# octaviogarcia/RaytracingOneWeekend

Hardware: AMD Instinct MI355X
Metric: Msamples/s (W×H×spp/s) + achieved HBM GB/s, 1080p@512spp traced scene (higher is better)
Workload: dtype f32; 1 GPU; C1 S-traced 1920x1080, 10496 spp timed (128 spp/step), depth 50; width=1920, height=1080, max_depth=50, parallelism=tile1, gather=RCCL send/recv (om_gather_frame), rccl_library=/usr/local/lib/python3.10/dist-packages/torch/lib/librccl.so, kernel=auto, pipeline=auto, tail_bounce=default, streams=2

## Files before the change

### raytracingoneweekend_amd/csrc/om_deal.h

```cpp
#pragma once
#include <cstdint>

#if defined(__HIPCC__) || defined(__CUDACC__)
#define OM_DEAL_HD __host__ __device__
#else
#define OM_DEAL_HD
#endif

struct Deal {
    uint64_t paths;
    uint64_t blocks;
    uint32_t nseg;
    uint32_t d;

    OM_DEAL_HD uint64_t groups() const { return (blocks + d - 1u) / d; }
    OM_DEAL_HD uint32_t blocks_of(uint32_t g) const {
        const uint64_t ng = groups();
        if (g >= ng) return 0u;
        const uint64_t mine = (ng - 1u - g) / nseg + 1u;
        uint64_t b = mine * d;
        if ((ng - 1u) % nseg == g) b -= ng * d - blocks;
        return (uint32_t)b;
    }
    OM_DEAL_HD uint64_t block(uint32_t g, uint32_t c) const {
        return ((uint64_t)(c / d) * nseg + g) * d + c % d;
    }
    OM_DEAL_HD uint32_t paths_of(uint32_t g) const {
        uint64_t n = (uint64_t)blocks_of(g) * 64u;
        if (blocks && ((blocks - 1u) / d) % nseg == g) n -= blocks * 64u - paths;
        return (uint32_t)n;
    }
    OM_DEAL_HD uint32_t capacity() const {
        return (uint32_t)((groups() + nseg - 1u) / nseg * d * 64u);
    }
};

inline uint32_t deal_segments(uint64_t max_paths, uint32_t cus, uint32_t lanes_per_cu, uint32_t blk, uint32_t spb) {
    const uint64_t want = (max_paths + blk - 1u) / blk, cap = (uint64_t)cus * (lanes_per_cu / blk);
    const uint32_t nseg = (uint32_t)(want < cap ? want : cap);
    return (nseg + spb - 1u) / spb * spb;
}

OM_DEAL_HD inline Deal make_deal(uint64_t paths, uint32_t nseg, uint32_t d) {
    return Deal{paths, (paths + 63u) / 64u, nseg, d};
}
```

### raytracingoneweekend_amd/csrc/om_tuning.h

```cpp
#pragma once

#ifndef OM_WF_BLOCK
#define OM_WF_BLOCK 512
#endif
#ifndef OM_WF_WAVES
#define OM_WF_WAVES 8
#endif
#ifndef OM_WF_TAIL_SPB
#define OM_WF_TAIL_SPB 2
#endif
#ifndef OM_WF_TAIL_WGS_PER_CU
#define OM_WF_TAIL_WGS_PER_CU 1
#endif
#ifndef OM_WF_MAX_PATHS_LOG2
#define OM_WF_MAX_PATHS_LOG2 27
#endif
#ifndef OM_WF_BATCH_SPP
#define OM_WF_BATCH_SPP 16
#endif
#ifndef OM_WF_MIN_PATHS_LOG2
#define OM_WF_MIN_PATHS_LOG2 25
#endif
#ifndef OM_WF_HYB_BYTES
#define OM_WF_HYB_BYTES 16384
#endif
#ifndef OM_WF_HYBW_BYTES
#define OM_WF_HYBW_BYTES 0
#endif
#ifndef OM_WF_HYB4_BYTES
#define OM_WF_HYB4_BYTES 0
#endif
#ifndef OM_WF_REFILL
#define OM_WF_REFILL 16
#endif
#ifndef OM_WF_TAIL_SHADE
#define OM_WF_TAIL_SHADE 1
#endif
#ifndef OM_WF_TAIL_UNROLL
#define OM_WF_TAIL_UNROLL 24
#endif
#ifndef OM_WF_TAIL_MARCH_WAVES
#define OM_WF_TAIL_MARCH_WAVES 8
#endif
#ifndef OM_WF_TAIL_REFILL
#define OM_WF_TAIL_REFILL OM_WF_REFILL
#endif
#ifndef OM_WF_TAIL_MARCHED
#define OM_WF_TAIL_MARCHED 1
#endif
#ifndef OM_MARCH_UNROLL
#define OM_MARCH_UNROLL 8
#endif
#ifndef OM_WF_ADAPTIVE_BATCHES
#define OM_WF_ADAPTIVE_BATCHES 3
#endif
#ifndef OM_WF_ADAPTIVE_PATHS_LOG2
#define OM_WF_ADAPTIVE_PATHS_LOG2 22
#endif
#ifndef OM_WF_ADAPTIVE_CAP_LOG2
#define OM_WF_ADAPTIVE_CAP_LOG2 26
#endif
#ifndef OM_WF_ADAPTIVE_TAIL
#define OM_WF_ADAPTIVE_TAIL 8
#endif
#ifndef OM_WF_LANES_PER_CU
#define OM_WF_LANES_PER_CU 2048
#endif
#ifndef OM_WF_LANES_PER_CU_WIDE
#define OM_WF_LANES_PER_CU_WIDE 8192
#endif
#ifndef OM_WF_DEAL_BLOCKS
#define OM_WF_DEAL_BLOCKS 8
#endif
#ifndef OM_WF_FUSE_B1
#define OM_WF_FUSE_B1 1
#endif
#ifndef OM_ACC_GROUP
#define OM_ACC_GROUP 8
#endif
#ifndef OM_B2_NODE_STRIDE
#define OM_B2_NODE_STRIDE 80
#endif
#ifndef OM_BARY_TREE_MIN
#define OM_BARY_TREE_MIN 16
#endif
#ifndef OM_SLAB_REACH
#define OM_SLAB_REACH 8192.0f
#endif
#ifndef OM_SPHERE_REACH
#define OM_SPHERE_REACH 16.0
#endif
```

### raytracingoneweekend_amd/csrc/om_wavefront.hip

```cpp
#include "om_wavefront.h"

#include <algorithm>
#include <type_traits>

#include "om_device.h"
#include "om_trace.h"
#include "om_tuning.h"
#include "om_deal.h"

using namespace omd;

namespace omw {

void QueueSet::release() {
    for (int a = 0; a < 2; ++a) {
        for (int b = 0; b < 3; ++b) { if (q[a][b]) (void)hipFree(q[a][b]); q[a][b] = nullptr; }
        if (qr[a]) (void)hipFree(qr[a]); qr[a] = nullptr;
    }
    if (res) (void)hipFree(res);
    if (res_id) (void)hipFree(res_id);
    if (counts) (void)hipFree(counts);
    if (hit) (void)hipFree(hit);
    res = nullptr; res_id = nullptr; counts = nullptr; hit = nullptr;
}

void Buffers::release() {
    for (auto& s : set) s.release();
    if (n0) (void)hipFree(n0);
    n0 = nullptr; n0_cap = 0;
    for (auto& st : side) { if (st) (void)hipStreamDestroy(st); st = nullptr; }

    for (auto e : ev) (void)hipEventDestroy(e);
    ev.clear();
    cap = 0; counts_n = 0; nsets = 0;
}

namespace {

constexpr uint32_t kNoSample = 0xFFFFFFFFu;
enum { TR_BRUTE = 1, TR_CULLED = 2, TR_BVH = 3, TR_SBVH_LDS = 4, TR_SBVH_GLOBAL = 5, TR_BVH2_LDS = 6, TR_BVH2_GLOBAL = 7,
       TR_BVH4_LDS = 8, TR_BVH4_GLOBAL = 9,
       TR_BVH2_WIDE = 10,
       TR_BARY = 16 };
constexpr int tr_base(int tr) { return tr & (TR_BARY - 1); }
constexpr bool tr_bary(int tr) { return (tr & TR_BARY) != 0; }
#define OM_WAVES_ATTR __attribute__((amdgpu_waves_per_eu(OM_WF_WAVES, OM_WF_WAVES)))
constexpr int kBlk = OM_WF_BLOCK;
constexpr int kStackDepth = 24;
constexpr uint32_t kB2Stride = OM_B2_NODE_STRIDE;
static_assert(kB2Stride % 16u == 0u && kB2Stride >= sizeof(OmBvh2Node), "16-B aligned node slots");
static_assert(kB2LdsBudget / sizeof(OmBvh2Node) * (kB2Stride / 16u) < OM_LEAF, "scaled BVH2 child codes stay below OM_LEAF");
template <int TR>
__host__ __device__ inline uint32_t stack_bytes(const OmSceneDev& S) {
    if (tr_base(TR) == TR_BVH2_WIDE) return kBlk * S.b2w_stack * 4u;
    return kBlk * ((tr_base(TR) == TR_BVH4_LDS || tr_base(TR) == TR_BVH4_GLOBAL) ? S.b4_stack : S.b2_stack) * 2u;
}
__host__ __device__ inline uint32_t b2_stage_bytes(const OmSceneDev& S) {
    return (S.n_b2nodes * kB2Stride + S.n_b2leaves * 4u + 15u) & ~15u;
}
constexpr uint32_t kTailSpb = OM_WF_TAIL_SPB;
constexpr uint32_t kTailWgsPerCu = OM_WF_TAIL_WGS_PER_CU;
constexpr uint32_t kWaves = kBlk / 64;
static_assert(kBlk % 64 == 0 && kTailWgsPerCu >= 1u, "whole waves; a tail grid");
constexpr bool kFuseB1 = OM_WF_FUSE_B1 != 0;
constexpr uint32_t kTailDefault = 16;
constexpr uint32_t kTailMarched = OM_WF_TAIL_MARCHED;
constexpr uint32_t kTailL2 = 10;
constexpr uint32_t kTailBigBatch = 24;
__host__ __device__ inline uint32_t hyb_nodes(const OmSceneDev& S) {
    constexpr uint32_t kCap = OM_WF_HYB_BYTES / (uint32_t)sizeof(OmBvh2NodeH);
    return S.b2_lds_bytes ? 0u : (S.n_b2nodes < kCap ? S.n_b2nodes : kCap);
}
static_assert(sizeof(OmBvh2NodeW) == sizeof(OmBvh2NodeH), "wide and half nodes share a buffer");
__host__ __device__ inline const OmBvh2NodeW* wide_nodes(const OmSceneDev& S) { return (const OmBvh2NodeW*)(S.b2h + S.n_b2nodes); }
__host__ __device__ inline uint32_t hybw_nodes(const OmSceneDev& S) {
    constexpr uint32_t kCap = OM_WF_HYBW_BYTES / (uint32_t)sizeof(OmBvh2NodeW);
    return S.n_b2wnodes < kCap ? S.n_b2wnodes : kCap;
}
__host__ __device__ inline uint32_t hyb4_nodes(const OmSceneDev& S) {
    constexpr uint32_t kCap = OM_WF_HYB4_BYTES / (uint32_t)sizeof(OmBvh4NodeH);
    return S.b4_lds_bytes ? 0u : (S.n_b4nodes < kCap ? S.n_b4nodes : kCap);
}
using MarchedC2Lds = MarchedExactLds<2, 1, 1>;
enum { MV_ARRAYS = 0, MV_EXACT_C2_LDS = 1 };
template <int TR>
__host__ __device__ constexpr bool exact_view_built() { return TR == TR_BRUTE || TR == TR_BVH2_LDS; }
__host__ __device__ inline Deal batch_deal(uint64_t paths, uint32_t nseg) { return make_deal(paths, nseg, OM_WF_DEAL_BLOCKS); }

extern __shared__ __attribute__((aligned(16))) uint4 wf_lds[];

__device__ __forceinline__ uint32_t wave_sum32(uint32_t v) {
#pragma unroll
    for (int off = 32; off > 0; off >>= 1) v += __shfl_xor(v, off, 64);
    return v;
}
__device__ __forceinline__ void flush_counter(unsigned long long* ctr, int slot, uint32_t v) {
    v = wave_sum32(v);
    if (__lane_id() == 0 && v) atomicAdd(&ctr[slot], (unsigned long long)v);
}

struct Seg {
    uint32_t nseg;
    uint32_t segcap;
};

struct AdPlan { uint32_t c, done; };
struct AdCfg {
    uint32_t sample_count;
    uint32_t batches;
    uint32_t paths;
};
__host__ __device__ inline uint32_t ad_batch(uint32_t c, uint32_t done, uint32_t j, const AdCfg& A) {
    if (c == 0u || done >= A.sample_count || j >= A.batches) return 0u;
    const uint32_t rem = A.sample_count - done, left = A.batches - j;
    const uint32_t even = (rem + left - 1u) / left, want = A.paths / c;
    const uint32_t b = even > want ? even : want;
    return b < rem ? b : rem;
// ... 27 lines not shown

struct Path {
    F3 o, d, cur;
    float depthf;
    uint32_t first_id, seg, slot;
    Rng g;
};

template <class V>
__device__ __forceinline__ V ld4(const V* q) {
    V v;
    v.x = __builtin_nontemporal_load(&q->x); v.y = __builtin_nontemporal_load(&q->y);
    v.z = __builtin_nontemporal_load(&q->z); v.w = __builtin_nontemporal_load(&q->w);
    return v;
}
__device__ __forceinline__ void load_ray(const Queue& Q, uint64_t i, Path& p) {
    const float4 a = ld4(Q.q0 + i), b = ld4(Q.q1 + i);
    p.o = f3(a.x, a.y, a.z); p.depthf = a.w;
    p.d = f3(b.x, b.y, b.z); p.first_id = __float_as_uint(b.w);
}
__device__ __forceinline__ void load_rest(const Queue& Q, uint64_t i, Path& p) {
    const float4 c = ld4(Q.q2 + i);
    const uint4 r = ld4(Q.qr + i);
    p.cur = f3(c.x, c.y, c.z); p.seg = __float_as_uint(c.w);
    p.g.s = r.x; p.g.k = r.y; p.slot = r.z;
}
template <class V>
__device__ __forceinline__ void st4(V* q, V v) {
    __builtin_nontemporal_store(v.x, &q->x); __builtin_nontemporal_store(v.y, &q->y);
    __builtin_nontemporal_store(v.z, &q->z); __builtin_nontemporal_store(v.w, &q->w);
}
__device__ __forceinline__ void store_path(const Queue& Q, uint64_t i, const Path& p) {
    st4(Q.q0 + i, make_float4(p.o.x, p.o.y, p.o.z, p.depthf));
    st4(Q.q1 + i, make_float4(p.d.x, p.d.y, p.d.z, __uint_as_float(p.first_id)));
    st4(Q.q2 + i, make_float4(p.cur.x, p.cur.y, p.cur.z, __uint_as_float(p.seg)));
    st4(Q.qr + i, make_uint4(p.g.s, p.g.k, p.slot, 0u));
}

struct Tracer {
    const OmBvh2Node* b2n;
    const OmBvh2NodeH* h2l;
    const OmBvh2NodeH* h2g;
    uint32_t nl;
    const OmBvh2NodeW* w2l;
    const OmBvh2NodeW* w2g;
    uint32_t* stk32;
    const OmBvh4Node* b4n;
    const OmBvh4NodeH* h4l;
    const OmBvh4NodeH* h4g;
    const uint32_t* bl;
    const OmAffineTest* recs;
    uint16_t* stk;
};

template <int TRF, uint32_t STACKS = 1>
__device__ __forceinline__ Tracer stage_scene(const OmSceneDev& S) {
    constexpr int TR = tr_base(TRF);
    Tracer t;
    t.stk = (uint16_t*)wf_lds + threadIdx.x;
    t.b2n = S.b2nodes; t.b4n = S.b4nodes; t.bl = S.b2leaves; t.recs = S.srecs;
    t.h2l = S.b2h; t.h2g = S.b2h; t.nl = 0;
    t.h4l = S.b4h; t.h4g = S.b4h;
    t.w2l = wide_nodes(S); t.w2g = wide_nodes(S); t.stk32 = (uint32_t*)wf_lds + threadIdx.x;
    if (TR == TR_BVH4_GLOBAL && hyb4_nodes(S)) {
        t.nl = hyb4_nodes(S);
        uint4* dst = wf_lds + STACKS * stack_bytes<TR>(S) / 16u;
        const uint4* sn = (const uint4*)S.b4h;
        for (uint32_t i = threadIdx.x; i < t.nl * (uint32_t)(sizeof(OmBvh4NodeH) / 16u); i += kBlk) dst[i] = sn[i];
        __syncthreads();
        t.h4l = (const OmBvh4NodeH*)dst;
    }
    if (TR == TR_BVH2_WIDE && hybw_nodes(S)) {
        t.nl = hybw_nodes(S);
        uint4* dst = wf_lds + STACKS * stack_bytes<TR>(S) / 16u;
        const uint4* sn = (const uint4*)wide_nodes(S);
        for (uint32_t i = threadIdx.x; i < t.nl * (uint32_t)(sizeof(OmBvh2NodeW) / 16u); i += kBlk) dst[i] = sn[i];
        __syncthreads();
        t.w2l = (const OmBvh2NodeW*)dst;
    }
    if (TR == TR_BVH2_GLOBAL && hyb_nodes(S)) {
        t.nl = hyb_nodes(S);
        uint4* dst = wf_lds + STACKS * stack_bytes<TR>(S) / 16u;
        const uint4* sn = (const uint4*)S.b2h;
        for (uint32_t i = threadIdx.x; i < t.nl * (uint32_t)(sizeof(OmBvh2NodeH) / 16u); i += kBlk) dst[i] = sn[i];
        __syncthreads();
        t.h2l = (const OmBvh2NodeH*)dst;
    }
    if (TR == TR_BVH2_LDS || TR == TR_BVH4_LDS) {
        constexpr uint32_t wn = TR == TR_BVH2_LDS ? (uint32_t)(sizeof(OmBvh2Node) / 16u) : (uint32_t)(sizeof(OmBvh4Node) / 16u);
        constexpr uint32_t ws = TR == TR_BVH2_LDS ? kB2Stride / 16u : wn;
        const uint32_t nn = (TR == TR_BVH2_LDS ? S.n_b2nodes : S.n_b4nodes) * wn;
        const uint4* sn = TR == TR_BVH2_LDS ? (const uint4*)S.b2nodes : (const uint4*)S.b4nodes;
        uint4* dst = wf_lds + STACKS * stack_bytes<TR>(S) / 16u;
        for (uint32_t i = threadIdx.x; i < nn; i += kBlk) {
            uint4 v = sn[i];
            if (TR == TR_BVH2_LDS && (i % wn) % 2u == 0u && v.w < OM_LEAF) v.w *= ws;
            dst[(i / wn) * ws + i % wn] = v;
        }
        uint32_t* ldst = (uint32_t*)(dst + nn / wn * ws);
        for (uint32_t i = threadIdx.x; i < S.n_b2leaves; i += kBlk) ldst[i] = S.b2leaves[i];
        __syncthreads();
        t.b2n = (const OmBvh2Node*)dst; t.b4n = (const OmBvh4Node*)dst; t.bl = ldst;
    }
    return t;
}

// ... 44 lines not shown
    } else {
        const float t = 0.5f * (p.d.y + 1.0f);
        p.cur = mul(p.cur, f3((1.0f - t) + 0.5f * t, (1.0f - t) + 0.7f * t, (1.0f - t) + 1.0f * t));
        seg_depth = INFINITY; seg_id = 0u;
    }
    bool finished = false;
    F3 result = p.cur;
    float rdepth = 0.0f; uint32_t rid = 0;
    if (p.seg == 0u) {
        p.depthf = seg_depth; p.first_id = seg_id;
        if (isinf(seg_depth)) { finished = true; rdepth = INFINITY; rid = 0u; }
    } else if (isinf(seg_depth)) {
        finished = true; rdepth = p.depthf; rid = p.first_id;
    }
    if (!finished && p.seg + 1u >= depth_cap) {
        finished = true; result = f3(-0.0f, -0.0f, -0.0f); rdepth = p.depthf; rid = p.first_id;
    }
    if (finished) {
        res[p.slot] = make_float4(result.x, result.y, result.z, rdepth);
        res_id[p.slot] = rid;
        return false;
    }
    p.seg += 1u;
    return true;
}

__device__ __forceinline__ bool gen_path(const OmParamsDev& P, const Gen& R, uint32_t stride, uint64_t i, Path& p,
                                         uint32_t& pixel, uint32_t* __restrict__ res_id) {
    const uint32_t s_local = (uint32_t)i / stride, kk = (uint32_t)i - s_local * stride;
    const uint32_t k = R.ad.list ? R.ad.list[kk] : kk;
    pixel = R.pixels[k];
    uint32_t s;
    bool live;
    if (R.n0) {
        const uint32_t v = R.n0[k];
        s = (v & 0x7FFFFFFFu) + R.done + s_local;
        live = s < P.spp_total && !(v >> 31);
    } else {
        const om_pixel_stats& ps = R.stats[R.by_pixel ? pixel : k];
        s = ps.n + s_local;
        live = s < P.spp_total && !(P.adaptive && (ps.flags & 1u));
    }
    if (!live) {
        res_id[i] = kNoSample;
        return false;
    }
    p.g = path_rng(P.skey, pixel, s);
    const uint32_t line = pixel / P.width;
    gen_camera_ray(R.C, P, R.jitter, (float)(pixel - P.width * line), (float)line, s, p.g, p.o, p.d);
    p.cur = f3(1.0f, 1.0f, 1.0f); p.depthf = 0.0f; p.first_id = 0u; p.seg = 0u; p.slot = (uint32_t)i;
    return true;
}

template <int TR, bool COUNT, bool MARCH, bool FIRST, bool HIT = false, bool USER = MARCH>
__global__ __launch_bounds__(kBlk) OM_WAVES_ATTR void k_bounce(OmSceneDev S, OmParamsDev P, Seg G, Gen R, Queue in,
                                                 const uint32_t* __restrict__ count_in, Queue out,
                                                 uint32_t* __restrict__ count_out, float4* __restrict__ res,
                                                 uint32_t* __restrict__ res_id, unsigned long long* __restrict__ counters,
                                                 const float2* __restrict__ hitbuf, uint32_t* __restrict__ tail_next) {
    constexpr bool FUSE = FIRST && !MARCH && !HIT && kFuseB1;
    const uint64_t seg0 = (uint64_t)blockIdx.x * G.segcap;
    uint32_t n, stride = R.n_pixels;
    Deal dl{};
    if (FIRST) {
        if (tail_next && blockIdx.x == 0 && threadIdx.x == 0) *tail_next = 0u;
        uint64_t paths = (uint64_t)R.n_pixels * R.batch;
        if (R.ad.list) {
            const AdPlan pl = uniform_load(R.ad.plan);
            stride = pl.c;
            paths = (uint64_t)pl.c * ad_batch(pl.c, pl.done, R.ad.j, R.ad.A);
        }
        dl = batch_deal(paths, G.nseg);
        n = dl.blocks_of(blockIdx.x);
    } else {
        n = count_in[blockIdx.x];
    }
    if (n == 0) {
        if (threadIdx.x == 0) count_out[blockIdx.x] = 0u;
        return;
    }
    __shared__ uint32_t q_next, q_out;
    if (threadIdx.x == 0) { q_next = kBlk / 64u; q_out = 0u; }
    __syncthreads();
    const Tracer T = HIT ? Tracer{} : stage_scene<TR>(S);
    const uint32_t depth_cap = P.max_depth > 1u ? P.max_depth : 1u;
    WorkT<COUNT, false, tr_bary(TR)> w;
    uint32_t segs = 0;
    const uint32_t lane = __lane_id();
    const uint32_t chunks = FIRST ? n : (n + 63u) / 64u;
    for (uint32_t chunk = __builtin_amdgcn_readfirstlane(threadIdx.x >> 6); chunk < chunks;) {
        const uint64_t i = FUSE  ? (uint64_t)((uint32_t)(dl.block(blockIdx.x, chunk) * 64u) + lane)
                         : FIRST ? dl.block(blockIdx.x, chunk) * 64u + lane : seg0 + chunk * 64u + lane;
        bool keep = false;
        Path p;
        uint32_t p_pixel = 0;
        if (FIRST ? i < dl.paths : chunk * 64u + lane < n) {
            if (FIRST) {
                uint32_t st = stride;
                if (FUSE) asm volatile("" : "+s"(st));
                keep = gen_path(P, R, st, i, p, p_pixel, res_id);
            } else {
                load_ray(in, i, p);
                load_rest(in, i, p);
                keep = true;
            }
        }
        float closest = 0.0f;
        int best = -1;
        const bool listed = FIRST && !HIT && (tr_base(TR) == TR_BVH2_LDS || tr_base(TR) == TR_BVH2_GLOBAL || tr_base(TR) == TR_BVH2_WIDE) && R.tile_off;
        if (listed && keep) {
            const uint32_t line = p_pixel / P.width;
            const uint32_t tile = (p_pixel - line * P.width) / 8u + (line / 8u) * P.tiles_x;
            closest = P.tmax;
            const uint32_t t0 = __builtin_amdgcn_readfirstlane(tile);
            if (__ballot(tile != t0) == 0)
                best = traced_tiles<true>(S, R.tile_off, R.tile_idx, t0, p.o, p.d, P.tmin, closest, w, R.tile_tnear);
            else
                best = traced_tiles(S, R.tile_off, R.tile_idx, tile, p.o, p.d, P.tmin, closest, w);
            if (MARCH) {
                float tm;
                const int mg = march(S, p.o, p.d, P.tmin, P.tmax, closest, P.march_steps, tm, w);
                if (mg >= 0) { best = mg; closest = tm; }
            }
        }
#pragma clang loop unroll(disable)
        for (uint32_t sg = 0u;; ++sg) {
            if (keep) {
                if (HIT) {
                    const float2 h = hitbuf[i];
                    closest = h.x; best = __float_as_int(h.y);
                } else if (!(listed && sg == 0u)) {
                    best = trace<TR, MARCH>(S, P, T, p.o, p.d, closest, w);
                }
                keep = shade_path<MARCH, USER>(S, P, depth_cap, p, closest, best, res, res_id);
                if (COUNT) segs++;
            }
            if (!FUSE || sg == 1u || __ballot(keep) == 0) break;
        }
        const uint64_t m = __ballot(keep);
        uint32_t obase = 0u, nc = 0u;
        if (lane == 0) {
            obase = m ? atomicAdd(&q_out, (uint32_t)__popcll(m)) : 0u;
            nc = atomicAdd(&q_next, 1u);
        }
        obase = __builtin_amdgcn_readfirstlane(obase);
        chunk = __builtin_amdgcn_readfirstlane(nc);
        const uint32_t rank = FUSE ? __builtin_amdgcn_mbcnt_hi((uint32_t)(m >> 32), __builtin_amdgcn_mbcnt_lo((uint32_t)m, 0u))
                                   : (uint32_t)__popcll(m & ((1ull << lane) - 1ull));
        if (keep) store_path(out, seg0 + obase + rank, p);
// ... 193 lines not shown
        if (__ballot(have || !dry) == 0) break;
    }
    return segs;
}

template <int TR, bool COUNT, int VIEW = MV_ARRAYS, uint32_t SPB = kTailSpb>
__global__ __launch_bounds__(kBlk) __attribute__((amdgpu_waves_per_eu(OM_WF_TAIL_MARCH_WAVES, OM_WF_TAIL_MARCH_WAVES)))
void k_tail_march(OmSceneDev S, OmParamsDev P, Seg G, Queue in,
                                               const uint32_t* __restrict__ count_in, float4* __restrict__ res,
                                               uint32_t* __restrict__ res_id, unsigned long long* __restrict__ counters) {
    __shared__ uint32_t pre[SPB + 1];
    __shared__ uint32_t next;
    const uint32_t s0 = blockIdx.x * SPB;
    if (threadIdx.x == 0) {
        uint32_t acc = 0;
        for (uint32_t k = 0; k < SPB; ++k) {
            pre[k] = acc;
            acc += s0 + k < G.nseg ? count_in[s0 + k] : 0u;
        }
        pre[SPB] = acc;
        next = kBlk;
    }
    __syncthreads();
    const uint32_t total = pre[SPB];
    if (total == 0) return;
    const Tracer T = stage_scene<TR>(S);
    const TailSrc src{in, pre, s0, SPB, G.segcap};
    WorkT<COUNT, false, tr_bary(TR)> w;
    uint32_t segs = 0;
    if constexpr (VIEW == MV_EXACT_C2_LDS) {
        __shared__ MarchedC2Lds::Block mblock;
        segs = tail_march_lanes<TR, COUNT>(S, P, T, MarchedC2Lds(S, &mblock), src, total, next, res, res_id, w);
    } else {
        segs = tail_march_lanes<TR, COUNT>(S, P, T, MarchedArrays(S), src, total, next, res, res_id, w);
    }
    if (COUNT) {
        flush_counter(counters, OMC_SEGMENTS, segs);
        flush_counter(counters, OMC_PRIM_TESTS, w.prim);
        flush_counter(counters, OMC_PRE_TESTS, w.pre);
        flush_counter(counters, OMC_MARCH, w.march);
    }
}

template <int TR, bool COUNT>
__global__ __launch_bounds__(kBlk) OM_WAVES_ATTR
void k_tail(OmSceneDev S, OmParamsDev P, Seg G, Queue in, const uint32_t* __restrict__ count_in, uint32_t pre_off,
            uint32_t* __restrict__ next, float4* __restrict__ res, uint32_t* __restrict__ res_id,
            unsigned long long* __restrict__ counters) {
    uint32_t* pre = (uint32_t*)wf_lds + pre_off / 4u;
    __shared__ uint32_t wave_sum[kWaves];
    const uint32_t lane = __lane_id(), wave = threadIdx.x >> 6;
    const uint32_t per = (G.nseg + kBlk - 1u) / kBlk;
    const uint32_t c0 = threadIdx.x * per, c1 = c0 + per < G.nseg ? c0 + per : G.nseg;
    uint32_t mine = 0;
    for (uint32_t k = c0; k < c1; ++k) mine += count_in[k];
    uint32_t incl = mine;
#pragma unroll
    for (int off = 1; off < 64; off <<= 1) {
        const uint32_t v = __shfl_up(incl, off, 64);
        if (lane >= (uint32_t)off) incl += v;
    }
    if (lane == 63u) wave_sum[wave] = incl;
    __syncthreads();
    uint32_t acc = incl - mine, total = 0;
#pragma unroll
    for (uint32_t k = 0; k < kWaves; ++k) {
        const uint32_t v = wave_sum[k];
        if (k < wave) acc += v;
        total += v;
    }
    if (total == 0) return;
    for (uint32_t k = c0; k < c1; ++k) { pre[k] = acc; acc += count_in[k]; }
    if (threadIdx.x == 0) pre[G.nseg] = total;
    __syncthreads();
    const Tracer T = stage_scene<TR>(S);
    const uint32_t depth_cap = P.max_depth > 1u ? P.max_depth : 1u;
    const TailSrc src{in, pre, 0u, G.nseg, G.segcap};
    WorkT<COUNT, false, tr_bary(TR)> w;
    uint32_t segs = 0;
    const uint32_t lanes = gridDim.x * kBlk;
    const uint32_t round = (wave + kWaves - blockIdx.x % kWaves) % kWaves;
    uint32_t idx = (round * gridDim.x + blockIdx.x) * 64u + lane;
    bool have = idx < total;
    bool more = total > lanes;
    Path p;
    if (have) src.load(idx, p);
    for (;;) {
        if (have) {
            float closest;
            const int best = trace<TR, false>(S, P, T, p.o, p.d, closest, w);
            if (COUNT) segs++;
            have = shade_path<false>(S, P, depth_cap, p, closest, best, res, res_id);
        }
        if (more) {
            const uint64_t want = __ballot(!have);
            if (want) {
                const uint32_t nw = (uint32_t)__popcll(want);
                uint32_t base = 0u;
                if (lane == 0) base = atomicAdd(next, nw);
                base = lanes + __builtin_amdgcn_readfirstlane(base);
                if (!have) {
                    idx = base + (uint32_t)__popcll(want & ((1ull << lane) - 1ull));
                    have = idx < total;
                    if (have) src.load(idx, p);
                }
                more = base + nw < total;
            }
        }
        if (__ballot(have) == 0) break;
    }
    if (COUNT) {
        flush_counter(counters, OMC_SEGMENTS, segs);
        flush_counter(counters, OMC_PRIM_TESTS, w.prim);
        flush_counter(counters, OMC_PRE_TESTS, w.pre);
        flush_counter(counters, OMC_MARCH, w.march);
    }
}

__device__ __forceinline__ bool window_edge(float tmin, float tmax) { return !(tmin >= 0.0f) || tmax != tmax; }
__device__ __forceinline__ bool far_origin(const OmSceneDev& S, F3 o) {
    if (S.n_bvh_nodes == 0) return false;
    const OmBvhNode N = S.bvh[0];
    const float dx = fmaxf(N.lo[0] - o.x, o.x - N.hi[0]), dy = fmaxf(N.lo[1] - o.y, o.y - N.hi[1]), dz = fmaxf(N.lo[2] - o.z, o.z - N.hi[2]);
// ... 232 lines not shown
                                                 uint32_t plan_stride) {
    const uint32_t k = blockIdx.x * kAdInitBlk + threadIdx.x;
    bool live = false;
    if (k < n_pixels) {
        const om_pixel_stats& ps = stats[by_pixel ? pixels[k] : k];
        live = !(ps.flags & 1u) && ps.n < spp_total;
    }
    const uint32_t s = (k >> 6) % ns;
    const uint64_t m = __ballot(live);
    uint32_t base = 0u;
    __shared__ uint32_t wg_n[4], wg_base[4];
    if (threadIdx.x < 4u) wg_n[threadIdx.x] = 0u;
    __syncthreads();
    if (__lane_id() == 0 && m) base = atomicAdd(&wg_n[s], (uint32_t)__popcll(m));
    __syncthreads();
    if (threadIdx.x < ns && wg_n[threadIdx.x])
        wg_base[threadIdx.x] = atomicAdd(&plans[(uint64_t)threadIdx.x * plan_stride].c, wg_n[threadIdx.x]);
    __syncthreads();
    base = __builtin_amdgcn_readfirstlane(base) + (m ? wg_base[s] : 0u);
    if (live) lists[s * list_stride + base + (uint32_t)__popcll(m & ((1ull << __lane_id()) - 1ull))] = k;
}

hipError_t grow(Buffers& B, uint64_t cap, uint32_t counts_n, int nsets) {
    hipError_t e;
    if (cap > B.cap || nsets > B.nsets) {
        for (auto& s : B.set) s.release();
        B.cap = 0; B.nsets = 0; B.counts_n = 0;
        for (int k = 0; k < nsets; ++k) {
            QueueSet& S = B.set[k];
            for (int a = 0; a < 2; ++a) {
                for (int b = 0; b < 3; ++b) if ((e = hipMalloc(&S.q[a][b], cap * sizeof(float4))) != hipSuccess) return e;
                if ((e = hipMalloc(&S.qr[a], cap * sizeof(uint4))) != hipSuccess) return e;
            }
            if ((e = hipMalloc(&S.res, cap * sizeof(float4))) != hipSuccess) return e;
            if ((e = hipMalloc(&S.res_id, cap * sizeof(uint32_t))) != hipSuccess) return e;
            if ((e = hipMalloc(&S.hit, cap * sizeof(float2))) != hipSuccess) return e;
        }
        B.cap = cap; B.nsets = nsets;
    }
    if (counts_n > B.counts_n) {
        for (int k = 0; k < B.nsets; ++k) {
            QueueSet& S = B.set[k];
            if (S.counts) (void)hipFree(S.counts);
            S.counts = nullptr;
            if ((e = hipMalloc(&S.counts, (size_t)counts_n * sizeof(uint32_t))) != hipSuccess) return e;
        }
        B.counts_n = counts_n;
    }
    return hipSuccess;
}

Queue queue(QueueSet& B, int k) { return Queue{B.q[k][0], B.q[k][1], B.q[k][2], B.qr[k]}; }

inline uint32_t tail_pre_off(uint32_t lds) { return (lds + 15u) & ~15u; }
inline uint32_t tail_lds(uint32_t lds, uint32_t nseg) { return tail_pre_off(lds) + (nseg + 1u) * 4u; }

inline uint32_t count_rows(uint32_t depth_cap) { return std::max<uint32_t>(depth_cap, kFuseB1 ? 2u : 1u) + 1u; }

template <int TR, bool COUNT, bool MARCH>
uint32_t run_batch(QueueSet& B, const Launch& L, hipStream_t st, Seg G, const Gen& R, uint32_t depth_cap,
                   uint32_t tail_at, uint32_t lds, uint32_t tail_grid) {
    Timer& tm = *L.timer;
    const bool each = tm.mode == 1;
    uint32_t launches = 0;
    const bool exact = MARCH && L.S.n_msdf == 0u && MarchedC2Lds::matches(L.S.n_msph, L.S.n_mbox, L.S.n_mtor);
    uint32_t* const tail_next = B.counts + (size_t)count_rows(depth_cap) * G.nseg;
    auto tail = [&](const Queue& in, const uint32_t* cin) {
        const int ti = each ? tm.begin(st) : -1;
        if constexpr (MARCH) {
            const uint32_t grid = (G.nseg + kTailSpb - 1u) / kTailSpb;
            if (exact && exact_view_built<TR>())
                hipLaunchKernelGGL((k_tail_march<TR, COUNT, exact_view_built<TR>() ? MV_EXACT_C2_LDS : MV_ARRAYS>), dim3(grid),
                                   dim3(kBlk), lds, st, L.S, L.P, G, in, cin, B.res, B.res_id, L.counters);
            else
                hipLaunchKernelGGL((k_tail_march<TR, COUNT>), dim3(grid), dim3(kBlk), lds, st, L.S, L.P, G, in, cin,
                                   B.res, B.res_id, L.counters);
        } else {
            hipLaunchKernelGGL((k_tail<TR, COUNT>), dim3(tail_grid), dim3(kBlk), tail_lds(lds, G.nseg), st, L.S, L.P, G, in, cin,
                               tail_pre_off(lds), tail_next, B.res, B.res_id, L.counters);
        }
        tm.end(ti, OM_KT_TAIL, st);
        return launches + 1u;
    };
    if constexpr (MARCH) {
        {
            const int ti = each ? tm.begin(st) : -1;
            hipLaunchKernelGGL((k_raygen<COUNT>), dim3(G.nseg), dim3(kBlk), 0, st, L.P, G, R, queue(B, 0), B.counts, B.res_id);
            tm.end(ti, OM_KT_BOUNCE0, st);
            ++launches;
        }
        for (uint32_t bounce = 0; bounce < depth_cap; ++bounce) {
            const Queue in = queue(B, bounce & 1u), out = queue(B, (bounce + 1u) & 1u);
            const uint32_t* cin = B.counts + (size_t)bounce * G.nseg;
            if (bounce >= tail_at) return tail(in, cin);
            uint32_t* cout = B.counts + (size_t)(bounce + 1u) * G.nseg;
            const int kc = bounce == 0 ? OM_KT_BOUNCE0 : OM_KT_BOUNCE;
            int ti = each ? tm.begin(st) : -1;
            if (exact && exact_view_built<TR>())
                hipLaunchKernelGGL((k_march<TR, COUNT, exact_view_built<TR>() ? MV_EXACT_C2_LDS : MV_ARRAYS>), dim3(G.nseg),
                                   dim3(kBlk), lds, st, L.S, L.P, G, in, cin, B.hit, L.counters);
            else
                hipLaunchKernelGGL((k_march<TR, COUNT, MV_ARRAYS>), dim3(G.nseg), dim3(kBlk), lds, st, L.S, L.P, G, in, cin,
                                   B.hit, L.counters);
            tm.end(ti, kc, st);
            ti = each ? tm.begin(st) : -1;
            if (exact && exact_view_built<TR>())
                hipLaunchKernelGGL((k_bounce<TR, COUNT, MARCH, false, true, false>), dim3(G.nseg), dim3(kBlk), 0, st, L.S, L.P, G,
                                   R, in, cin, out, cout, B.res, B.res_id, L.counters, (const float2*)B.hit, (uint32_t*)nullptr);
            else
                hipLaunchKernelGGL((k_bounce<TR, COUNT, MARCH, false, true>), dim3(G.nseg), dim3(kBlk), 0, st, L.S, L.P, G, R, in,
                                   cin, out, cout, B.res, B.res_id, L.counters, (const float2*)B.hit, (uint32_t*)nullptr);
            tm.end(ti, kc, st);
            launches += 2u;
        }
        return launches;
    } else {
    for (uint32_t bounce = 0, next; bounce < depth_cap; bounce = next) {
        next = bounce + (bounce == 0 && kFuseB1 ? 2u : 1u);
        const Queue in = queue(B, bounce & 1u), out = queue(B, next & 1u);
        const uint32_t* cin = B.counts + (size_t)bounce * G.nseg;
        if (bounce > 0 && bounce >= tail_at) return tail(in, cin);
        uint32_t* cout = B.counts + (size_t)next * G.nseg;
        const int ti = each ? tm.begin(st) : -1;
        if (bounce == 0)
            hipLaunchKernelGGL((k_bounce<TR, COUNT, MARCH, true>), dim3(G.nseg), dim3(kBlk), lds, st, L.S, L.P, G, R, in,
                               cin, out, cout, B.res, B.res_id, L.counters, (const float2*)nullptr, tail_next);
        else
            hipLaunchKernelGGL((k_bounce<TR, COUNT, MARCH, false>), dim3(G.nseg), dim3(kBlk), lds, st, L.S, L.P, G, R, in,
                               cin, out, cout, B.res, B.res_id, L.counters, (const float2*)nullptr, (uint32_t*)nullptr);
        tm.end(ti, bounce == 0 ? OM_KT_BOUNCE0 : OM_KT_BOUNCE, st);
        ++launches;
    }
    return launches;
    }
}

template <int TR>
uint32_t run_tr(bool count, bool march, QueueSet& B, const Launch& L, hipStream_t st, Seg G, const Gen& R,
                uint32_t depth_cap, uint32_t tail_at, uint32_t lds, uint32_t tail_grid) {
    if (count && march) return run_batch<TR, true, true>(B, L, st, G, R, depth_cap, tail_at, lds, tail_grid);
    if (count) return run_batch<TR, true, false>(B, L, st, G, R, depth_cap, tail_at, lds, tail_grid);
    if (march) return run_batch<TR, false, true>(B, L, st, G, R, depth_cap, tail_at, lds, tail_grid);
    return run_batch<TR, false, false>(B, L, st, G, R, depth_cap, tail_at, lds, tail_grid);
}

hipError_t ensure_events(Buffers& B, size_t n) {
    while (B.ev.size() < n) {
        hipEvent_t e = nullptr;
        const hipError_t r = hipEventCreateWithFlags(&e, hipEventDisableTiming);
        if (r != hipSuccess) return r;
        B.ev.push_back(e);
    }
    return hipSuccess;
}

int pick_trace(int trace_mode, const OmSceneDev& S) {
    int tr = trace_mode == TR_SBVH_LDS ? TR_SBVH_GLOBAL : trace_mode;
    if (tr == TR_BVH2_WIDE) {
        if (S.n_b2wnodes) return TR_BVH2_WIDE | TR_BARY;
        tr = TR_BVH2_LDS;
    }
    if (tr == TR_BVH4_LDS) tr = S.n_b4nodes == 0 ? TR_BVH2_LDS : (S.b4_lds_bytes ? TR_BVH4_LDS : TR_BVH4_GLOBAL);
    if (tr == TR_BVH2_LDS && S.n_b2nodes == 0 && S.n_b2wnodes) return TR_BVH2_WIDE | TR_BARY;
    if (tr == TR_BVH2_LDS)
        tr = S.n_b2nodes == 0 ? (S.n_bvh_nodes <= 1u ? TR_BRUTE : TR_BVH) : (S.b2_lds_bytes ? TR_BVH2_LDS : TR_BVH2_GLOBAL);
    const int bary = S.n_srec_bary ? TR_BARY : 0;
    switch (tr) {
        case TR_BRUTE: case TR_CULLED: case TR_BVH: return tr;
        case TR_SBVH_GLOBAL: case TR_BVH2_LDS: case TR_BVH4_LDS: case TR_BVH4_GLOBAL: return tr | bary;
        default: return TR_BVH2_GLOBAL | bary;
    }
}
uint32_t trace_lds(int trf, const OmSceneDev& S) {
    const int tr = tr_base(trf);
    return tr == TR_BVH2_LDS ? stack_bytes<TR_BVH2_LDS>(S) + b2_stage_bytes(S)
         : tr == TR_BVH2_GLOBAL ? stack_bytes<TR_BVH2_GLOBAL>(S) + hyb_nodes(S) * (uint32_t)sizeof(OmBvh2NodeH)
         : tr == TR_BVH4_LDS ? stack_bytes<TR_BVH4_LDS>(S) + S.b4_lds_bytes
         : tr == TR_BVH4_GLOBAL ? stack_bytes<TR_BVH4_GLOBAL>(S) + hyb4_nodes(S) * (uint32_t)sizeof(OmBvh4NodeH)
         : tr == TR_BVH2_WIDE ? stack_bytes<TR_BVH2_WIDE>(S) + hybw_nodes(S) * (uint32_t)sizeof(OmBvh2NodeW)
         : 0u;
}
template <class F>
void with_tr(int tr, F f) {
    switch (tr) {
        case TR_BRUTE: f(std::integral_constant<int, TR_BRUTE>{}); break;
        case TR_CULLED: f(std::integral_constant<int, TR_CULLED>{}); break;
        case TR_BVH: f(std::integral_constant<int, TR_BVH>{}); break;
        case TR_SBVH_GLOBAL: f(std::integral_constant<int, TR_SBVH_GLOBAL>{}); break;
        case TR_BVH2_LDS: f(std::integral_constant<int, TR_BVH2_LDS>{}); break;
        case TR_BVH4_LDS: f(std::integral_constant<int, TR_BVH4_LDS>{}); break;
        case TR_BVH4_GLOBAL: f(std::integral_constant<int, TR_BVH4_GLOBAL>{}); break;
        case TR_SBVH_GLOBAL | TR_BARY: f(std::integral_constant<int, TR_SBVH_GLOBAL | TR_BARY>{}); break;
        case TR_BVH2_LDS | TR_BARY: f(std::integral_constant<int, TR_BVH2_LDS | TR_BARY>{}); break;
        case TR_BVH2_GLOBAL | TR_BARY: f(std::integral_constant<int, TR_BVH2_GLOBAL | TR_BARY>{}); break;
        case TR_BVH4_LDS | TR_BARY: f(std::integral_constant<int, TR_BVH4_LDS | TR_BARY>{}); break;
        case TR_BVH4_GLOBAL | TR_BARY: f(std::integral_constant<int, TR_BVH4_GLOBAL | TR_BARY>{}); break;
        case TR_BVH2_WIDE | TR_BARY: f(std::integral_constant<int, TR_BVH2_WIDE | TR_BARY>{}); break;
        default: f(std::integral_constant<int, TR_BVH2_GLOBAL>{}); break;
    }
}

template <int TR, bool MARCH, bool USER>
void launch_query(const Query& Q, const OmParamsDev& P, uint32_t grid, uint32_t lds, hipStream_t st) {
    if (Q.windows) {
        if (Q.count)
            hipLaunchKernelGGL((k_query_windows<TR, MARCH, USER, true>), dim3(grid), dim3(kBlk), lds, st, Q.S, P, Q.rays, Q.windows, Q.n, Q.hits, Q.counters);
        else
            hipLaunchKernelGGL((k_query_windows<TR, MARCH, USER, false>), dim3(grid), dim3(kBlk), lds, st, Q.S, P, Q.rays, Q.windows, Q.n, Q.hits, Q.counters);
    } else if (Q.count)
        hipLaunchKernelGGL((k_query<TR, MARCH, USER, true>), dim3(grid), dim3(kBlk), lds, st, Q.S, P, Q.rays, Q.n, Q.hits, Q.counters);
    else
        hipLaunchKernelGGL((k_query<TR, MARCH, USER, false>), dim3(grid), dim3(kBlk), lds, st, Q.S, P, Q.rays, Q.n, Q.hits, Q.counters);
}
template <int TR, bool MARCH>
void launch_occluded(const Query& Q, const OmParamsDev& P, uint32_t grid, uint32_t lds, hipStream_t st) {
    if (Q.count)
        hipLaunchKernelGGL((k_occluded<TR, MARCH, true>), dim3(grid), dim3(kBlk), lds, st, Q.S, P, Q.rays, Q.windows, Q.n, Q.occluded, Q.counters);
    else
        hipLaunchKernelGGL((k_occluded<TR, MARCH, false>), dim3(grid), dim3(kBlk), lds, st, Q.S, P, Q.rays, Q.windows, Q.n, Q.occluded, Q.counters);
}

}

hipError_t render(Buffers& B, const Launch& L, hipStream_t st, std::string& err) {
    const uint32_t n_px = L.n_pixels;
    if (n_px == 0 || L.P.sample_count == 0) return hipSuccess;
    const bool adaptive = L.P.adaptive != 0u;
    const uint32_t want = std::max<uint32_t>(1u, std::min<uint32_t>(L.streams, (uint32_t)kMaxSets));
    const uint64_t kMaxPaths = std::min<uint64_t>(1ull << OM_WF_MAX_PATHS_LOG2,
                                                  std::max<uint64_t>(1ull << OM_WF_MIN_PATHS_LOG2, (uint64_t)OM_WF_BATCH_SPP * n_px));
    uint32_t ns, nb, batch = 0, ad_k = 0, cmax = 0;
    uint64_t max_paths;
    std::vector<uint32_t> done_at(1, 0u);
    AdCfg A{};
    if (adaptive) {
        const uint32_t chunks = (n_px + 63u) / 64u;
        ns = std::min<uint32_t>(want, chunks);
        cmax = std::min<uint32_t>(n_px, (chunks + ns - 1u) / ns * 64u);
        const uint64_t capmax = 1ull << OM_WF_ADAPTIVE_CAP_LOG2;
        uint64_t k = L.ad_batches ? L.ad_batches : OM_WF_ADAPTIVE_BATCHES;
        while (k < L.P.sample_count && (uint64_t)cmax * ((L.P.sample_count + k - 1u) / k) > capmax) ++k;
        ad_k = (uint32_t)std::min<uint64_t>(k, L.P.sample_count);
        A.sample_count = L.P.sample_count; A.batches = ad_k;
        A.paths = 1u << (L.ad_paths_log2 ? L.ad_paths_log2 : OM_WF_ADAPTIVE_PATHS_LOG2);
        max_paths = std::max<uint64_t>(std::min<uint64_t>(A.paths, (uint64_t)cmax * L.P.sample_count),
                                       (uint64_t)cmax * ((L.P.sample_count + ad_k - 1u) / ad_k));
        nb = ad_k * ns;
    } else {
        const bool concurrent = want >= 2u && L.P.sample_count >= 2u;
        batch = (uint32_t)std::max<uint64_t>(1, std::min<uint64_t>(L.P.sample_count, kMaxPaths / n_px));
        if (concurrent) batch = std::min<uint32_t>(batch, (L.P.sample_count + want - 1u) / want);
        while (done_at.back() < L.P.sample_count)
            done_at.push_back(done_at.back() + std::min(batch, L.P.sample_count - done_at.back()));
        nb = (uint32_t)done_at.size() - 1u;
        ns = concurrent ? std::min<uint32_t>(want, nb) : 1u;
        max_paths = (uint64_t)n_px * batch;
    }
    const uint32_t depth_cap = L.P.max_depth > 1u ? L.P.max_depth : 1u;
    int dev = 0;
    (void)hipGetDevice(&dev);
    int cus = 256;
    (void)hipDeviceGetAttribute(&cus, hipDeviceAttributeMultiprocessorCount, dev);
    const int tr = pick_trace(L.trace_mode, L.S);
    const bool march = (L.S.n_msph + L.S.n_mbox + L.S.n_mtor + L.S.n_msdf) != 0u;
    const bool l2_tree = tr_base(tr) == TR_BVH2_GLOBAL || tr_base(tr) == TR_BVH4_GLOBAL || tr_base(tr) == TR_BVH2_WIDE;
    const uint32_t tail_at = L.tail_bounce ? L.tail_bounce
                           : march ? kTailMarched
                           : (l2_tree ? kTailL2 : adaptive ? OM_WF_ADAPTIVE_TAIL
                              : max_paths > (1ull << 25) ? kTailBigBatch : kTailDefault) + (kFuseB1 ? 1u : 0u);
    const uint32_t lanes_per_cu = (march || l2_tree) ? OM_WF_LANES_PER_CU_WIDE : OM_WF_LANES_PER_CU;
    const uint32_t nseg = deal_segments(max_paths, (uint32_t)cus, lanes_per_cu, kBlk, kTailSpb);
    const uint32_t segcap = batch_deal(max_paths, nseg).capacity();
    hipError_t e = grow(B, (uint64_t)nseg * segcap, count_rows(depth_cap) * nseg + 1u, (int)ns);
    if (e != hipSuccess) { err = "wavefront buffer allocation failed"; return e; }
    const uint32_t lds = trace_lds(tr, L.S);
    const uint32_t tail_grid = (uint32_t)cus * kTailWgsPerCu;
    int lds_max = 0;
    (void)hipDeviceGetAttribute(&lds_max, hipDeviceAttributeMaxSharedMemoryPerBlock, dev);
    if (!march && tail_at < depth_cap && tail_lds(lds, nseg) > (uint32_t)lds_max) {
        err = "the tail's LDS request exceeds the device's limit";
        return hipErrorInvalidValue;
    }
    if (lds > (uint32_t)lds_max) {
        err = "the traversal's LDS request exceeds the device's limit";
        return hipErrorInvalidValue;
    }
    Gen R;
    R.C = L.C; R.jitter = L.jitter; R.stats = L.stats; R.pixels = L.pixels; R.n_pixels = n_px;
    R.by_pixel = L.stats_by_pixel ? 1u : 0u;
    R.tile_off = L.tile_off; R.tile_idx = L.tile_idx; R.tile_tnear = L.tile_tnear;
    R.n0 = nullptr; R.done = 0; R.ad = AdList{};
    hipStream_t streams[kMaxSets] = {st, st, st, st};
    Timer& tm = *L.timer;
    const int call_ti = tm.begin(st);
    const uint32_t plan_stride = ad_k + 1u;
    const uint64_t words = adaptive ? (uint64_t)ns * 2u * cmax + (uint64_t)ns * plan_stride * 2u : (ns > 1 ? n_px : 0u);
    if (words > B.n0_cap) {
        if (B.n0) (void)hipFree(B.n0);
        B.n0 = nullptr; B.n0_cap = 0;
        if ((e = hipMalloc(&B.n0, (size_t)words * sizeof(uint32_t))) != hipSuccess) { err = "n0 allocation failed"; return e; }
        B.n0_cap = words;
    }
    uint32_t* lists = B.n0;
    AdPlan* plans = adaptive ? (AdPlan*)(B.n0 + (uint64_t)ns * 2u * cmax) : nullptr;
    if (adaptive) {
        (void)hipMemsetAsync(plans, 0, (size_t)ns * plan_stride * sizeof(AdPlan), st);
        hipLaunchKernelGGL(k_ad_init, dim3((n_px + kAdInitBlk - 1u) / kAdInitBlk), dim3(kAdInitBlk), 0, st, L.stats, L.pixels, n_px, R.by_pixel,
                           L.P.spp_total, ns, lists, (uint64_t)2u * cmax, plans, plan_stride);
    } else if (ns > 1) {
        hipLaunchKernelGGL(k_snapshot, dim3((n_px + 255u) / 256u), dim3(256), 0, st, L.stats, L.pixels, n_px, R.by_pixel, B.n0);
        R.n0 = B.n0;
    }
    if (ns > 1) {
        if ((e = ensure_events(B, kMaxSets + nb)) != hipSuccess) { err = "event creation failed"; return e; }
        (void)hipEventRecord(B.ev[0], st);
        for (uint32_t k = 1; k < ns; ++k) {
            if (!B.side[k] && (e = hipStreamCreateWithFlags(&B.side[k], hipStreamNonBlocking)) != hipSuccess) {
                err = "side stream creation failed"; return e;
            }
            streams[k] = B.side[k];
            (void)hipStreamWaitEvent(streams[k], B.ev[0], 0);
        }
    }
    uint32_t launches = 0;
    for (uint32_t i = 0; i < nb; ++i) {
        const uint32_t sidx = i % ns;
        hipStream_t si = streams[sidx];
        QueueSet& QS = B.set[sidx];
        Seg G;
        G.nseg = nseg;
        uint32_t b = 0, grid_a;
        AdList ad{};
        if (adaptive) {
            const uint32_t j = i / ns;
            uint32_t* lbase = lists + (uint64_t)sidx * 2u * cmax;
// ... 88 lines not shown
```

Before: 8102 Msamples/s.

## Rebalance later-bounce work across workgroups by dealing 64-path chunks evenly

For early non-first bounces (up to OM_WF_DEAL_LATER launches), each workgroup no longer processes only its own segment's queue. Every block now scans all segment counts, splits the total number of 64-path chunks evenly across blocks, and builds an LDS list of the source segments it covers. It then walks that list with a cursor while processing. The aim is to remove the load imbalance that appears as paths terminate unevenly across segments. In exchange, every block does a redundant scan over all segment counts, uses extra LDS, and loses locality between its input segment and its output segment.

New measurement: 7927 Msamples/s. 2.2% lower.

```diff
diff --git a/raytracingoneweekend_amd/csrc/om_deal.h b/raytracingoneweekend_amd/csrc/om_deal.h
--- a/raytracingoneweekend_amd/csrc/om_deal.h
+++ b/raytracingoneweekend_amd/csrc/om_deal.h
@@ -5,6 +5,11 @@
 #define OM_DEAL_HD __host__ __device__
 #else
 #define OM_DEAL_HD
+#endif
+#if defined(__HIP_DEVICE_COMPILE__)
+#define OM_DEAL_UNIFORM(x) ((uint32_t)__builtin_amdgcn_readfirstlane((int)(x)))
+#else
+#define OM_DEAL_UNIFORM(x) ((uint32_t)(x))
 #endif
 
 struct Deal {
@@ -44,3 +49,32 @@
 OM_DEAL_HD inline Deal make_deal(uint64_t paths, uint32_t nseg, uint32_t d) {
     return Deal{paths, (paths + 63u) / 64u, nseg, d};
 }
+
+OM_DEAL_HD inline uint32_t later_chunks(uint32_t count) { return (count + 63u) / 64u; }
+OM_DEAL_HD inline uint32_t later_slots(uint32_t segcap) { return segcap / 64u + 1u; }
+constexpr uint32_t kLaterMaxSeg = 65536u;
+
+struct LaterDeal {
+    uint32_t chunks;
+    uint32_t nseg;
+    OM_DEAL_HD uint32_t first(uint32_t g) const { return (uint32_t)((uint64_t)g * chunks / nseg); }
+    OM_DEAL_HD uint32_t share(uint32_t g) const { return first(g + 1u) - first(g); }
+    OM_DEAL_HD static bool touches(uint32_t e, uint32_t count, uint32_t lo, uint32_t hi) {
+        return count != 0u && e < hi && e + later_chunks(count) > lo;
+    }
+};
+
+struct LaterCursor {
+    uint32_t k, seg, base, count;
+    OM_DEAL_HD void start(const uint16_t* list, const uint32_t* counts, uint32_t base0) {
+        k = 0u; seg = OM_DEAL_UNIFORM(list[0]); base = base0; count = OM_DEAL_UNIFORM(counts[seg]);
+    }
+    OM_DEAL_HD uint32_t seek(const uint16_t* list, const uint32_t* counts, uint32_t c) {
+        while (c - base >= later_chunks(count)) {
+            base += later_chunks(count);
+            seg = OM_DEAL_UNIFORM(list[++k]); count = OM_DEAL_UNIFORM(counts[seg]);
+        }
+        return c - base;
+    }
+    OM_DEAL_HD uint32_t live(uint32_t cis) const { return count - cis * 64u < 64u ? count - cis * 64u : 64u; }
+};
diff --git a/raytracingoneweekend_amd/csrc/om_tuning.h b/raytracingoneweekend_amd/csrc/om_tuning.h
--- a/raytracingoneweekend_amd/csrc/om_tuning.h
+++ b/raytracingoneweekend_amd/csrc/om_tuning.h
@@ -75,6 +75,9 @@
 #ifndef OM_WF_FUSE_B1
 #define OM_WF_FUSE_B1 1
 #endif
+#ifndef OM_WF_DEAL_LATER
+#define OM_WF_DEAL_LATER 15
+#endif
 #ifndef OM_ACC_GROUP
 #define OM_ACC_GROUP 8
 #endif
diff --git a/raytracingoneweekend_amd/csrc/om_wavefront.hip b/raytracingoneweekend_amd/csrc/om_wavefront.hip
--- a/raytracingoneweekend_amd/csrc/om_wavefront.hip
+++ b/raytracingoneweekend_amd/csrc/om_wavefront.hip
@@ -63,6 +63,7 @@
 constexpr uint32_t kWaves = kBlk / 64;
 static_assert(kBlk % 64 == 0 && kTailWgsPerCu >= 1u, "whole waves; a tail grid");
 constexpr bool kFuseB1 = OM_WF_FUSE_B1 != 0;
+constexpr uint32_t kDealLater = OM_WF_DEAL_LATER;
 constexpr uint32_t kTailDefault = 16;
 constexpr uint32_t kTailMarched = OM_WF_TAIL_MARCHED;
 constexpr uint32_t kTailL2 = 10;
@@ -196,6 +197,17 @@
     const OmAffineTest* recs;
     uint16_t* stk;
 };
+
+template <int TR>
+__host__ __device__ inline uint32_t stage_lds(const OmSceneDev& S) {
+    return TR == TR_BVH2_LDS ? stack_bytes<TR_BVH2_LDS>(S) + b2_stage_bytes(S)
+         : TR == TR_BVH2_GLOBAL ? stack_bytes<TR_BVH2_GLOBAL>(S) + hyb_nodes(S) * (uint32_t)sizeof(OmBvh2NodeH)
+         : TR == TR_BVH4_LDS ? stack_bytes<TR_BVH4_LDS>(S) + S.b4_lds_bytes
+         : TR == TR_BVH4_GLOBAL ? stack_bytes<TR_BVH4_GLOBAL>(S) + hyb4_nodes(S) * (uint32_t)sizeof(OmBvh4NodeH)
+         : TR == TR_BVH2_WIDE ? stack_bytes<TR_BVH2_WIDE>(S) + hybw_nodes(S) * (uint32_t)sizeof(OmBvh2NodeW)
+         : 0u;
+}
+__host__ __device__ inline uint32_t tail_pre_off(uint32_t lds) { return (lds + 15u) & ~15u; }
 
 template <int TRF, uint32_t STACKS = 1>
 __device__ __forceinline__ Tracer stage_scene(const OmSceneDev& S) {
@@ -346,16 +358,41 @@
     return true;
 }
 
-template <int TR, bool COUNT, bool MARCH, bool FIRST, bool HIT = false, bool USER = MARCH>
+__device__ __forceinline__ uint32_t block_scan(uint32_t mine, uint32_t* wave_sum, uint32_t& total) {
+    const uint32_t lane = __lane_id(), wave = threadIdx.x >> 6;
+    uint32_t incl = mine;
+#pragma unroll
+    for (int off = 1; off < 64; off <<= 1) {
+        const uint32_t v = __shfl_up(incl, off, 64);
+        if (lane >= (uint32_t)off) incl += v;
+    }
+    if (lane == 63u) wave_sum[wave] = incl;
+    __syncthreads();
+    uint32_t acc = incl - mine;
+    total = 0;
+#pragma unroll
+    for (uint32_t k = 0; k < kWaves; ++k) {
+        const uint32_t v = wave_sum[k];
+        if (k < wave) acc += v;
+        total += v;
+    }
+    return acc;
+}
+
+template <int TR, bool COUNT, bool MARCH, bool FIRST, bool HIT = false, bool USER = MARCH, bool DEAL = false>
 __global__ __launch_bounds__(kBlk) OM_WAVES_ATTR void k_bounce(OmSceneDev S, OmParamsDev P, Seg G, Gen R, Queue in,
                                                  const uint32_t* __restrict__ count_in, Queue out,
                                                  uint32_t* __restrict__ count_out, float4* __restrict__ res,
                                                  uint32_t* __restrict__ res_id, unsigned long long* __restrict__ counters,
                                                  const float2* __restrict__ hitbuf, uint32_t* __restrict__ tail_next) {
     constexpr bool FUSE = FIRST && !MARCH && !HIT && kFuseB1;
+    static_assert(!DEAL || (!FIRST && !MARCH && !HIT), "the deal is the plain later-bounce form's");
     const uint64_t seg0 = (uint64_t)blockIdx.x * G.segcap;
     uint32_t n, stride = R.n_pixels;
     Deal dl{};
+    uint32_t* deal_base = nullptr;
+    uint16_t* deal_list = nullptr;
+    uint32_t deal_lo = 0;
     if (FIRST) {
         if (tail_next && blockIdx.x == 0 && threadIdx.x == 0) *tail_next = 0u;
         uint64_t paths = (uint64_t)R.n_pixels * R.batch;
@@ -366,6 +403,37 @@
         }
         dl = batch_deal(paths, G.nseg);
         n = dl.blocks_of(blockIdx.x);
+    } else if constexpr (DEAL) {
+        __shared__ uint32_t deal_sum[2][kWaves];
+        const uint32_t per = (G.nseg + kBlk - 1u) / kBlk;
+        const uint32_t c0 = threadIdx.x * per, c1 = c0 + per < G.nseg ? c0 + per : G.nseg;
+        uint32_t mine = 0, total;
+        for (uint32_t k = c0; k < c1; ++k) mine += later_chunks(count_in[k]);
+        const uint32_t e0 = block_scan(mine, deal_sum[0], total);
+        const LaterDeal ld{total, G.nseg};
+        deal_lo = ld.first(blockIdx.x);
+        n = ld.share(blockIdx.x);
+        if (n != 0) {
+            const uint32_t hi = deal_lo + n;
+            uint32_t e = e0, hits = 0, listed;
+            for (uint32_t k = c0; k < c1; ++k) {
+                const uint32_t c = count_in[k];
+                hits += LaterDeal::touches(e, c, deal_lo, hi) ? 1u : 0u;
+                e += later_chunks(c);
+            }
+            uint32_t at = block_scan(hits, deal_sum[1], listed);
+            deal_base = (uint32_t*)wf_lds + tail_pre_off(stage_lds<tr_base(TR)>(S)) / 4u;
+            deal_list = (uint16_t*)(deal_base + 1);
+            e = e0;
+            for (uint32_t k = c0; k < c1; ++k) {
+                const uint32_t c = count_in[k];
+                if (LaterDeal::touches(e, c, deal_lo, hi)) {
+                    if (at == 0u) *deal_base = e;
+                    deal_list[at++] = (uint16_t)k;
+                }
+                e += later_chunks(c);
+            }
+        }
     } else {
         n = count_in[blockIdx.x];
     }
@@ -381,14 +449,18 @@
     WorkT<COUNT, false, tr_bary(TR)> w;
     uint32_t segs = 0;
     const uint32_t lane = __lane_id();
-    const uint32_t chunks = FIRST ? n : (n + 63u) / 64u;
+    const uint32_t chunks = FIRST || DEAL ? n : (n + 63u) / 64u;
+    LaterCursor cur{};
+    if constexpr (DEAL) cur.start(deal_list, count_in, OM_DEAL_UNIFORM(*deal_base));
     for (uint32_t chunk = __builtin_amdgcn_readfirstlane(threadIdx.x >> 6); chunk < chunks;) {
+        const uint32_t cis = DEAL ? cur.seek(deal_list, count_in, deal_lo + chunk) : chunk;
         const uint64_t i = FUSE  ? (uint64_t)((uint32_t)(dl.block(blockIdx.x, chunk) * 64u) + lane)
-                         : FIRST ? dl.block(blockIdx.x, chunk) * 64u + lane : seg0 + chunk * 64u + lane;
+                         : FIRST ? dl.block(blockIdx.x, chunk) * 64u + lane
+                         : DEAL  ? (uint64_t)cur.seg * G.segcap + cis * 64u + lane : seg0 + chunk * 64u + lane;
         bool keep = false;
         Path p;
         uint32_t p_pixel = 0;
-        if (FIRST ? i < dl.paths : chunk * 64u + lane < n) {
+        if (FIRST ? i < dl.paths : DEAL ? lane < cur.live(cis) : chunk * 64u + lane < n) {
             if (FIRST) {
                 uint32_t st = stride;
                 if (FUSE) asm volatile("" : "+s"(st));
@@ -688,23 +760,9 @@
     const uint32_t lane = __lane_id(), wave = threadIdx.x >> 6;
     const uint32_t per = (G.nseg + kBlk - 1u) / kBlk;
     const uint32_t c0 = threadIdx.x * per, c1 = c0 + per < G.nseg ? c0 + per : G.nseg;
-    uint32_t mine = 0;
+    uint32_t mine = 0, total;
     for (uint32_t k = c0; k < c1; ++k) mine += count_in[k];
-    uint32_t incl = mine;
-#pragma unroll
-    for (int off = 1; off < 64; off <<= 1) {
-        const uint32_t v = __shfl_up(incl, off, 64);
-        if (lane >= (uint32_t)off) incl += v;
-    }
-    if (lane == 63u) wave_sum[wave] = incl;
-    __syncthreads();
-    uint32_t acc = incl - mine, total = 0;
-#pragma unroll
-    for (uint32_t k = 0; k < kWaves; ++k) {
-        const uint32_t v = wave_sum[k];
-        if (k < wave) acc += v;
-        total += v;
-    }
+    uint32_t acc = block_scan(mine, wave_sum, total);
     if (total == 0) return;
     for (uint32_t k = c0; k < c1; ++k) { pre[k] = acc; acc += count_in[k]; }
     if (threadIdx.x == 0) pre[G.nseg] = total;
@@ -1043,8 +1101,8 @@
 
 Queue queue(QueueSet& B, int k) { return Queue{B.q[k][0], B.q[k][1], B.q[k][2], B.qr[k]}; }
 
-inline uint32_t tail_pre_off(uint32_t lds) { return (lds + 15u) & ~15u; }
 inline uint32_t tail_lds(uint32_t lds, uint32_t nseg) { return tail_pre_off(lds) + (nseg + 1u) * 4u; }
+inline uint32_t deal_lds(uint32_t lds, uint32_t segcap) { return tail_pre_off(lds) + 4u + later_slots(segcap) * 2u; }
 
 inline uint32_t count_rows(uint32_t depth_cap) { return std::max<uint32_t>(depth_cap, kFuseB1 ? 2u : 1u) + 1u; }
 
@@ -1116,7 +1174,12 @@
         if (bounce == 0)
             hipLaunchKernelGGL((k_bounce<TR, COUNT, MARCH, true>), dim3(G.nseg), dim3(kBlk), lds, st, L.S, L.P, G, R, in,
                                cin, out, cout, B.res, B.res_id, L.counters, (const float2*)nullptr, tail_next);
-        else
+        else if (launches <= kDealLater) {
+            if constexpr (kDealLater != 0u)
+                hipLaunchKernelGGL((k_bounce<TR, COUNT, MARCH, false, false, MARCH, true>), dim3(G.nseg), dim3(kBlk),
+                                   deal_lds(lds, G.segcap), st, L.S, L.P, G, R, in, cin, out, cout, B.res, B.res_id, L.counters,
+                                   (const float2*)nullptr, (uint32_t*)nullptr);
+        } else
             hipLaunchKernelGGL((k_bounce<TR, COUNT, MARCH, false>), dim3(G.nseg), dim3(kBlk), lds, st, L.S, L.P, G, R, in,
                                cin, out, cout, B.res, B.res_id, L.counters, (const float2*)nullptr, (uint32_t*)nullptr);
         tm.end(ti, bounce == 0 ? OM_KT_BOUNCE0 : OM_KT_BOUNCE, st);
@@ -1163,13 +1226,14 @@
     }
 }
 uint32_t trace_lds(int trf, const OmSceneDev& S) {
-    const int tr = tr_base(trf);
-    return tr == TR_BVH2_LDS ? stack_bytes<TR_BVH2_LDS>(S) + b2_stage_bytes(S)
-         : tr == TR_BVH2_GLOBAL ? stack_bytes<TR_BVH2_GLOBAL>(S) + hyb_nodes(S) * (uint32_t)sizeof(OmBvh2NodeH)
-         : tr == TR_BVH4_LDS ? stack_bytes<TR_BVH4_LDS>(S) + S.b4_lds_bytes
-         : tr == TR_BVH4_GLOBAL ? stack_bytes<TR_BVH4_GLOBAL>(S) + hyb4_nodes(S) * (uint32_t)sizeof(OmBvh4NodeH)
-         : tr == TR_BVH2_WIDE ? stack_bytes<TR_BVH2_WIDE>(S) + hybw_nodes(S) * (uint32_t)sizeof(OmBvh2NodeW)
-         : 0u;
+    switch (tr_base(trf)) {
+        case TR_BVH2_LDS: return stage_lds<TR_BVH2_LDS>(S);
+        case TR_BVH2_GLOBAL: return stage_lds<TR_BVH2_GLOBAL>(S);
+        case TR_BVH4_LDS: return stage_lds<TR_BVH4_LDS>(S);
+        case TR_BVH4_GLOBAL: return stage_lds<TR_BVH4_GLOBAL>(S);
+        case TR_BVH2_WIDE: return stage_lds<TR_BVH2_WIDE>(S);
+        default: return 0u;
+    }
 }
 template <class F>
 void with_tr(int tr, F f) {
@@ -1272,6 +1336,12 @@
         err = "the tail's LDS request exceeds the device's limit";
         return hipErrorInvalidValue;
     }
+    const uint32_t later_at = kFuseB1 ? 2u : 1u;
+    if (kDealLater != 0u && !march && later_at < depth_cap && later_at < tail_at &&
+        (deal_lds(lds, segcap) > (uint32_t)lds_max || nseg > kLaterMaxSeg)) {
+        err = "the dealt bounce's LDS request exceeds the device's limit";
+        return hipErrorInvalidValue;
+    }
     if (lds > (uint32_t)lds_max) {
         err = "the traversal's LDS request exceeds the device's limit";
         return hipErrorInvalidValue;
```
